# phymhan/supervised-gan

Measured on AMD Instinct MI355X. Metric: train-step images/sec, fcgan 512x512 bs=1/GPU, higher is better.
Workload: dtype f32 (bf16x3 MFMA); 1 GPU; fcgan deconv-G(ngf32, z 8x8x8) + 3x PatchGAN-D(ndf32, n_layers 3, scale 1/2/4) 512x512 bs=1, n_update_D=1 n_update_G=2, Adam, pool 50 (BASELINE configs[1] shape, fp32 compute); synthetic batches resident in HBM (ring of 64); parallelism=dp1, global_batch=1, hip_graph=True, skip_wasted_D_wgrad=False

## Files before the change

supervised-gan_amd/csrc/sgan_ew.hip:

```cpp
#include "sgan_reduce.h"

thread_local char g_sgan_err[512] = {0};
thread_local const char* g_sgan_last_kernel = "";

int sgan_fail(int code, const char* fmt, ...) {
    va_list ap;
    va_start(ap, fmt);
    vsnprintf(g_sgan_err, sizeof(g_sgan_err), fmt, ap);
    va_end(ap);
    return code;
}

extern "C" const char* sgan_version(void) { return "sgan_hip 0.2 (gfx950; fp32 MFMA 16x16x4 + split-bf16 MFMA 32x32x16)"; }
extern "C" const char* sgan_last_error(void) { return g_sgan_err; }
extern "C" const char* sgan_last_kernel(void) { return g_sgan_last_kernel; }
extern "C" int sgan_stat_replicas(void) { return SGAN_STAT_REPLICAS; }
extern "C" int sgan_set_device(int32_t device_id) {
    hipError_t e = hipSetDevice(device_id);
    if (e != hipSuccess) {
        (void)hipGetLastError();
        return sgan_fail(SGAN_ERR_HIP, "hipSetDevice(%d): %s", (int)device_id, hipGetErrorString(e));
    }
    return SGAN_OK;
}
extern "C" int sgan_stream_device(void* stream, int32_t* device_id) {
    if (!device_id) return sgan_fail(SGAN_ERR_INVALID, "null device_id");
    hipDevice_t dev;
    hipError_t e = hipStreamGetDevice((hipStream_t)stream, &dev);
    if (e != hipSuccess) {
        (void)hipGetLastError();
        return sgan_fail(SGAN_ERR_HIP, "hipStreamGetDevice: %s", hipGetErrorString(e));
    }
    *device_id = (int32_t)dev;
    return SGAN_OK;
}

#define SG_PROF_MAX 8192
static bool g_prof_on = false;
static int g_prof_n = 0;
static hipEvent_t g_prof_e0[SG_PROF_MAX], g_prof_e1[SG_PROF_MAX];
static const char* g_prof_name[SG_PROF_MAX];
static bool g_prof_open = false;

void sg_prof_begin(hipStream_t st) {
    if (!g_prof_on || g_prof_n >= SG_PROF_MAX) return;
    if (hipEventCreate(&g_prof_e0[g_prof_n]) != hipSuccess || hipEventCreate(&g_prof_e1[g_prof_n]) != hipSuccess) return;
    (void)hipEventRecord(g_prof_e0[g_prof_n], st);
    g_prof_open = true;
}

void sg_prof_end(hipStream_t st, const char* name) {
    if (!g_prof_open) return;
    (void)hipEventRecord(g_prof_e1[g_prof_n], st);
    g_prof_name[g_prof_n] = name;
    ++g_prof_n;
    g_prof_open = false;
}

extern "C" int sgan_profile_enable(int on) {
    for (int i = 0; i < g_prof_n; ++i) {
        (void)hipEventDestroy(g_prof_e0[i]);
        (void)hipEventDestroy(g_prof_e1[i]);
    }
    g_prof_n = 0;
    g_prof_on = on != 0;
    return SGAN_OK;
}

extern "C" int sgan_profile_count(void) { return g_prof_n; }

extern "C" int sgan_profile_mark(void* stream) {
    sg_prof_begin((hipStream_t)stream);
    sg_prof_end((hipStream_t)stream, "null");
    return SGAN_OK;
}

extern "C" int sgan_profile_read(int i, const char** name, float* ms) {
    if (i < 0 || i >= g_prof_n || !name || !ms) return sgan_fail(SGAN_ERR_INVALID, "bad profile record index");
    *name = g_prof_name[i];
    if (hipEventElapsedTime(ms, g_prof_e0[i], g_prof_e1[i]) != hipSuccess) return sgan_fail(SGAN_ERR_HIP, "hipEventElapsedTime failed");
    return SGAN_OK;
}

struct SgNormBwdJob {
    float* dy; const float* x; const double* sums; float* dgamma; float* dbeta; unsigned* amax;
    SgNorm xn;
    int32_t dy_ld, x_ld, npix, C, sums_sq, sums_rep, blocks;
};
struct SgNormBwdTable { SgNormBwdJob j[8]; };

__global__ __launch_bounds__(256) void sg_norm_bwd_apply_kernel(const SgNormBwdTable T) {
    sg_warm_kernargs<(int)sizeof(SgNormBwdTable)>();
    const SgNormBwdJob& J = T.j[blockIdx.y];
    if ((int)blockIdx.x >= J.blocks) return;
    const int C = J.C;
    extern __shared__ __attribute__((aligned(16))) char smem[];
    float* cA = reinterpret_cast<float*>(smem);
    float* cMean = cA + C;
    float* cRstd = cMean + C;
    float* cS1 = cRstd + C;
    float* cS2 = cS1 + C;
    const double invM = 1.0 / (double)J.npix;
    for (int c = threadIdx.x; c < C; c += 256) {
        float mean, rstd;
        sg_mean_rstd(J.xn, C, c, mean, rstd);
        const float g = J.xn.gamma ? J.xn.gamma[c] : 1.f;
        cA[c] = g * rstd;
        cMean[c] = mean;
        cRstd[c] = rstd;
        const double s1 = sg_stat_sum(J.sums, c, J.sums_rep), s2 = sg_stat_sum(J.sums, J.sums_sq + c, J.sums_rep);
        cS1[c] = (float)(s1 * invM);
        cS2[c] = (float)(s2 * invM);
        if (blockIdx.x == 0) {
            if (J.dgamma) atomicAdd(&J.dgamma[c], (float)s2);
            if (J.dbeta) atomicAdd(&J.dbeta[c], (float)s1);
        }
    }
    SG_SYNC();
    const int CQ = C >> 2;
    const int64_t total = (int64_t)J.npix * CQ;
    float* dy = J.dy;
    const float* x = J.x;
    const int64_t stride = (int64_t)J.blocks * 256;
    float amax = 0.f;
    for (int64_t e0 = (int64_t)blockIdx.x * 256 + threadIdx.x; e0 < total; e0 += 4 * stride) {
        f32x4 d[4], xv[4];
        int64_t od[4];
        int cc[4];
#pragma unroll
        for (int u = 0; u < 4; ++u) {
            const int64_t e = e0 + u * stride;
            const bool ok = e < total;
            const int p = ok ? (int)(e / CQ) : 0;
            cc[u] = ok ? (int)(e - (int64_t)p * CQ) * 4 : 0;
            od[u] = ok ? (int64_t)p * J.dy_ld + cc[u] : -1;
            d[u] = *reinterpret_cast<const f32x4*>(dy + (ok ? od[u] : 0));
            xv[u] = *reinterpret_cast<const f32x4*>(x + (ok ? (int64_t)p * J.x_ld + cc[u] : 0));
        }
#pragma unroll
        for (int u = 0; u < 4; ++u) {
            if (od[u] < 0) continue;
            const int c = cc[u];
#pragma unroll
            for (int j = 0; j < 4; ++j) {
                const float xhat = (xv[u][j] - cMean[c + j]) * cRstd[c + j];
                d[u][j] = cA[c + j] * (d[u][j] - cS1[c + j] - xhat * cS2[c + j]);
                amax = fmaxf(amax, fabsf(d[u][j]));
            }
            *reinterpret_cast<f32x4*>(dy + od[u]) = d[u];
        }
    }
    if (J.amax) {
        for (int o = 32; o > 0; o >>= 1) amax = fmaxf(amax, __shfl_xor(amax, o));
        SG_SYNC();
        if ((threadIdx.x & 63) == 0) cA[threadIdx.x >> 6] = amax;
        SG_SYNC();
        if (threadIdx.x == 0) {
            const unsigned mine = __builtin_bit_cast(unsigned, fmaxf(fmaxf(cA[0], cA[1]), fmaxf(cA[2], cA[3])));
            if (mine > __hip_atomic_load(J.amax, __ATOMIC_RELAXED, __HIP_MEMORY_SCOPE_AGENT)) atomicMax(J.amax, mine);
        }
    }
}

extern "C" int sgan_norm_bwd_apply_multi(const sgan_norm_bwd_job* jobs, int32_t n, void* stream) {
    SGAN_CHECK(jobs && n >= 1 && n <= 8, "1..8 jobs");
    SgNormBwdTable T;
    int maxb = 1, maxC = 4;
    for (int i = 0; i < n; ++i) {
        const sgan_norm_bwd_job& S = jobs[i];
        SGAN_CHECK(S.dy && S.x && S.x_norm && S.x_norm->stats && S.bwd_sums, "null argument in job %d", i);
        SGAN_CHECK((S.C & 3) == 0 && S.C > 0 && S.C <= 4096 && S.dy_ld >= S.C && S.x_ld >= S.C && (S.dy_ld & 3) == 0 &&
                       (S.x_ld & 3) == 0 && S.npix > 0, "bad dims in job %d", i);
        SgNormBwdJob& J = T.j[i];
        J.dy = S.dy; J.x = S.x; J.sums = S.bwd_sums; J.dgamma = S.dgamma; J.dbeta = S.dbeta;
        J.amax = reinterpret_cast<unsigned*>(S.amax_out);
        J.xn = sg_norm_from(S.x_norm);
        J.dy_ld = S.dy_ld; J.x_ld = S.x_ld; J.npix = S.npix; J.C = S.C;
        J.sums_sq = S.bwd_sums_sq_stride ? S.bwd_sums_sq_stride : S.C;
        J.sums_rep = S.bwd_sums_rep_stride;
        const int64_t total = (int64_t)S.npix * (S.C >> 2);
        static const int chunk = getenv("SGAN_NBA_CHUNK") ? atoi(getenv("SGAN_NBA_CHUNK")) : 4;
        int blocks = sg_cdiv(total, 256 * (chunk > 0 ? chunk : 4));
        if (blocks > 2048) blocks = 2048;
        if (blocks < 1) blocks = 1;
        J.blocks = blocks;
        if (blocks > maxb) maxb = blocks;
        if (S.C > maxC) maxC = S.C;
    }
    hipLaunchKernelGGL(sg_norm_bwd_apply_kernel, dim3(maxb, n), dim3(256), (size_t)5 * maxC * 4, (hipStream_t)stream, T);
    SGAN_LAUNCH_CHECK();
    return SGAN_OK;
}

extern "C" int sgan_norm_bwd_apply(float* dy, int32_t dy_ld, const float* x, int32_t x_ld, int32_t npix, int32_t C,
                                   const sgan_norm_desc* x_norm, const double* bwd_sums, int32_t bwd_sums_sq_stride,
                                   float* dgamma, float* dbeta, void* stream) {
    sgan_norm_bwd_job j = {dy, dy_ld, x, x_ld, npix, C, x_norm, bwd_sums, bwd_sums_sq_stride, dgamma, dbeta, 0, nullptr};
    return sgan_norm_bwd_apply_multi(&j, 1, stream);
}

__global__ __launch_bounds__(256) void sg_norm_apply_fwd_kernel(const float* u, int u_ld, SgNorm un, const float* mask,
                                                                const float* noise, float sigma, float* t, int t_ld, int npix,
                                                                int C) {
    extern __shared__ __attribute__((aligned(16))) char smem[];
    float* cMean = reinterpret_cast<float*>(smem);
    float* cA = cMean + C;
    float* cB = cA + C;
    for (int c = threadIdx.x; c < C; c += 256) {
        float mean = 0.f, rstd = 1.f;
        if (un.stats) sg_mean_rstd(un, C, c, mean, rstd);
        cMean[c] = mean;
        cA[c] = (un.gamma ? un.gamma[c] : 1.f) * rstd;
        cB[c] = un.beta ? un.beta[c] : 0.f;
    }
    SG_SYNC();
    const int CQ = C >> 2;
    const int64_t total = (int64_t)npix * CQ;
    for (int64_t e = (int64_t)blockIdx.x * 256 + threadIdx.x; e < total; e += (int64_t)gridDim.x * 256) {
        const int p = (int)(e / CQ), c = (int)(e - (int64_t)p * CQ) * 4;
        const f32x4 x = *reinterpret_cast<const f32x4*>(u + (int64_t)p * u_ld + c);
        f32x4 m = (f32x4){1.f, 1.f, 1.f, 1.f}, nz = (f32x4){0.f, 0.f, 0.f, 0.f};
        if (mask) m = *reinterpret_cast<const f32x4*>(mask + (int64_t)p * C + c);
        if (noise) nz = *reinterpret_cast<const f32x4*>(noise + (int64_t)p * C + c);
        f32x4 o;
#pragma unroll
        for (int j = 0; j < 4; ++j) o[j] = ((x[j] - cMean[c + j]) * cA[c + j] + cB[c + j]) * m[j] + sigma * nz[j];
        *reinterpret_cast<f32x4*>(t + (int64_t)p * t_ld + c) = o;
    }
}

__global__ __launch_bounds__(256) void sg_norm_apply_bwd_sums_kernel(float* dt, int dt_ld, const float* mask, const float* u,
                                                                     int u_ld, SgNorm un, double* sums, int npix, int C) {
    extern __shared__ __attribute__((aligned(16))) char smem[];
    float* cMean = reinterpret_cast<float*>(smem);
    float* cRstd = cMean + C;
    float* red = cRstd + C;
    for (int c = threadIdx.x; c < C; c += 256) {
        float mean = 0.f, rstd = 1.f;
        if (un.stats) sg_mean_rstd(un, C, c, mean, rstd);
        cMean[c] = mean;
        cRstd[c] = rstd;
    }
    for (int i = threadIdx.x; i < 2 * C; i += 256) red[i] = 0.f;
    SG_SYNC();
    const int CQ = C >> 2;
    const int64_t total = (int64_t)npix * CQ;
    if (256 % CQ == 0) {
        const int c = (threadIdx.x % CQ) * 4;
        const f32x4 mean = *reinterpret_cast<const f32x4*>(cMean + c), rstd = *reinterpret_cast<const f32x4*>(cRstd + c);
        f32x4 s1 = (f32x4){0.f, 0.f, 0.f, 0.f}, s2 = s1;
        for (int64_t e = (int64_t)blockIdx.x * 256 + threadIdx.x; e < total; e += (int64_t)gridDim.x * 256) {
            const int64_t p = e / CQ;
            f32x4 d = *reinterpret_cast<const f32x4*>(dt + p * dt_ld + c);
            const f32x4 x = *reinterpret_cast<const f32x4*>(u + p * u_ld + c);
            if (mask) {
                d *= *reinterpret_cast<const f32x4*>(mask + p * C + c);
                *reinterpret_cast<f32x4*>(dt + p * dt_ld + c) = d;
            }
            s1 += d;
            s2 += d * ((x - mean) * rstd);
        }
#pragma unroll
        for (int j = 0; j < 4; ++j) {
            atomicAdd(&red[c + j], s1[j]);
            atomicAdd(&red[C + c + j], s2[j]);
        }
    } else {
        for (int64_t e = (int64_t)blockIdx.x * 256 + threadIdx.x; e < total; e += (int64_t)gridDim.x * 256) {
            const int p = (int)(e / CQ), c = (int)(e - (int64_t)p * CQ) * 4;
            f32x4 d = *reinterpret_cast<const f32x4*>(dt + (int64_t)p * dt_ld + c);
            const f32x4 x = *reinterpret_cast<const f32x4*>(u + (int64_t)p * u_ld + c);
            if (mask) {
                const f32x4 m = *reinterpret_cast<const f32x4*>(mask + (int64_t)p * C + c);
                d *= m;
                *reinterpret_cast<f32x4*>(dt + (int64_t)p * dt_ld + c) = d;
            }
#pragma unroll
            for (int j = 0; j < 4; ++j) {
                const float xhat = (x[j] - cMean[c + j]) * cRstd[c + j];
                atomicAdd(&red[c + j], d[j]);
                atomicAdd(&red[C + c + j], d[j] * xhat);
            }
        }
    }
    SG_SYNC();
    for (int c = threadIdx.x; c < C; c += 256) {
        atomicAdd(&sums[c], (double)red[c]);
        atomicAdd(&sums[C + c], (double)red[C + c]);
    }
}

extern "C" int sgan_norm_apply_fwd(const float* u, int32_t u_ld, const sgan_norm_desc* u_norm, const float* mask,
                                   const float* noise, float sigma, float* t, int32_t t_ld, int32_t npix, int32_t C, void* stream) {
    SGAN_CHECK(u && t && npix > 0 && C > 0 && (C & 3) == 0 && u_ld >= C && t_ld >= C && (u_ld & 3) == 0 && (t_ld & 3) == 0, "bad argument");
    const int64_t total = (int64_t)npix * (C >> 2);
    int blocks = sg_cdiv(total, 256 * 2);
    if (blocks > 2048) blocks = 2048;
    if (blocks < 1) blocks = 1;
    hipLaunchKernelGGL(sg_norm_apply_fwd_kernel, dim3(blocks), dim3(256), (size_t)3 * C * 4, (hipStream_t)stream, u, u_ld,
                       sg_norm_from(u_norm), mask, noise, sigma, t, t_ld, npix, C);
    SGAN_LAUNCH_CHECK();
    return SGAN_OK;
}

extern "C" int sgan_norm_apply_bwd_sums(float* dt, int32_t dt_ld, const float* mask, const float* u, int32_t u_ld,
                                        const sgan_norm_desc* u_norm, double* bwd_sums, int32_t npix, int32_t C, void* stream) {
    SGAN_CHECK(dt && u && bwd_sums && npix > 0 && C > 0 && (C & 3) == 0 && u_ld >= C && dt_ld >= C, "bad argument");
    const int64_t total = (int64_t)npix * (C >> 2);
    int blocks = sg_cdiv(total, 256 * 8);
    if (blocks > 512) blocks = 512;
    if (blocks < 1) blocks = 1;
    hipLaunchKernelGGL(sg_norm_apply_bwd_sums_kernel, dim3(blocks), dim3(256), (size_t)4 * C * 4, (hipStream_t)stream, dt, dt_ld,
                       mask, u, u_ld, sg_norm_from(u_norm), bwd_sums, npix, C);
    SGAN_LAUNCH_CHECK();
    return SGAN_OK;
}

__device__ __forceinline__ int sg_refl(int i, int n) { return i < 0 ? -i : (i >= n ? 2 * (n - 1) - i : i); }

__global__ __launch_bounds__(256) void sg_pad_reflect_fwd_kernel(const float* x, int x_ld, int H, int W, int C, SgNorm xn, const float* mask,
                                                                 int pad, float* out, int out_ld) {
    extern __shared__ __attribute__((aligned(16))) char smem[];
    float* cSc = reinterpret_cast<float*>(smem);
    float* cSh = cSc + C;
    for (int c = threadIdx.x; c < C; c += 256) {
        float sc = 1.f, sh = 0.f;
        if (xn.stats) {
            float mean, rstd;
            sg_mean_rstd(xn, C, c, mean, rstd);
            const float gm = xn.gamma ? xn.gamma[c] : 1.f, bt = xn.beta ? xn.beta[c] : 0.f;
            sc = gm * rstd;
            sh = bt - mean * sc;
        }
        cSc[c] = sc;
        cSh[c] = sh;
    }
    SG_SYNC();
    const int CQ = C >> 2, Wp = W + 2 * pad, Hp = H + 2 * pad;
    const int64_t total = (int64_t)Hp * Wp * CQ;
    for (int64_t e = (int64_t)blockIdx.x * 256 + threadIdx.x; e < total; e += (int64_t)gridDim.x * 256) {
        const int c = (int)(e % CQ) * 4;
        const int64_t pp = e / CQ;
        const int px = (int)(pp % Wp), py = (int)(pp / Wp);
        const int64_t src = (int64_t)sg_refl(py - pad, H) * W + sg_refl(px - pad, W);
        f32x4 v = *reinterpret_cast<const f32x4*>(x + src * x_ld + c);
#pragma unroll
        for (int j = 0; j < 4; ++j) v[j] = sg_act(v[j] * cSc[c + j] + cSh[c + j], xn.act, xn.slope);
        if (mask) v *= *reinterpret_cast<const f32x4*>(mask + src * C + c);
        *reinterpret_cast<f32x4*>(out + pp * out_ld + c) = v;
    }
}

extern "C" int sgan_pad_reflect_fwd(const float* x, int32_t x_ld, int32_t H, int32_t W, int32_t C, const sgan_norm_desc* x_norm,
                                    const float* mask, int32_t pad, float* out, int32_t out_ld, void* stream) {
    SGAN_CHECK(x && out && H > 0 && W > 0 && C > 0 && (C & 3) == 0 && (x_ld & 3) == 0 && (out_ld & 3) == 0 && x_ld >= C && out_ld >= C,
               "bad argument");
    SGAN_CHECK(pad >= 0 && pad < H && pad < W, "reflection padding must be smaller than the image");
    const int64_t total = (int64_t)(H + 2 * pad) * (W + 2 * pad) * (C >> 2);
    int blocks = sg_cdiv(total, 256 * 4);
    if (blocks > 2048) blocks = 2048;
    hipLaunchKernelGGL(sg_pad_reflect_fwd_kernel, dim3(blocks), dim3(256), (size_t)2 * C * 4, (hipStream_t)stream, x, x_ld, H, W, C,
                       sg_norm_from(x_norm), mask, pad, out, out_ld);
    SGAN_LAUNCH_CHECK();
    return SGAN_OK;
}

__global__ __launch_bounds__(256) void sg_pad_reflect_bwd_kernel(const float* dout, int dout_ld, int H, int W, int C, int pad, const float* x,
                                                                 int x_ld, SgNorm xn, const float* mask, float* din, int din_ld,
                                                                 double* sums, int sums_sq) {
    extern __shared__ __attribute__((aligned(16))) char smem[];
    float* cMean = reinterpret_cast<float*>(smem);
    float* cRstd = cMean + C;
    float* cG = cRstd + C;
    float* cB = cG + C;
    double* red = reinterpret_cast<double*>(cB + C);
    for (int c = threadIdx.x; c < C; c += 256) {
        float mean = 0.f, rstd = 1.f;
        if (xn.stats) sg_mean_rstd(xn, C, c, mean, rstd);
        cMean[c] = mean;
        cRstd[c] = rstd;
        cG[c] = (xn.stats && xn.gamma) ? xn.gamma[c] : 1.f;
        cB[c] = (xn.stats && xn.beta) ? xn.beta[c] : 0.f;
    }
    for (int i = threadIdx.x; i < 2 * C; i += 256) red[i] = 0.0;
    SG_SYNC();
    const int CQ = C >> 2, Wp = W + 2 * pad;
    const int64_t total = (int64_t)H * W * CQ;
    const bool has_x = x != nullptr;
    for (int64_t e = (int64_t)blockIdx.x * 256 + threadIdx.x; e < total; e += (int64_t)gridDim.x * 256) {
        const int c = (int)(e % CQ) * 4;
        const int64_t pix = e / CQ;
        const int xx = (int)(pix % W), yy = (int)(pix / W);
        int ys[3], xs[3], ny = 0, nx = 0;
        ys[ny++] = yy + pad;
        if (yy >= 1 && yy <= pad) ys[ny++] = pad - yy;
        if (yy <= H - 2 && yy >= H - 1 - pad) ys[ny++] = pad + 2 * (H - 1) - yy;
        xs[nx++] = xx + pad;
        if (xx >= 1 && xx <= pad) xs[nx++] = pad - xx;
        if (xx <= W - 2 && xx >= W - 1 - pad) xs[nx++] = pad + 2 * (W - 1) - xx;
        f32x4 d = (f32x4){0.f, 0.f, 0.f, 0.f};
        for (int a = 0; a < ny; ++a)
            for (int b = 0; b < nx; ++b) d += *reinterpret_cast<const f32x4*>(dout + ((int64_t)ys[a] * Wp + xs[b]) * dout_ld + c);
        if (mask) d *= *reinterpret_cast<const f32x4*>(mask + pix * C + c);
        if (has_x) {
            const f32x4 xv = *reinterpret_cast<const f32x4*>(x + pix * x_ld + c);
#pragma unroll
            for (int j = 0; j < 4; ++j) {
                const float xhat = (xv[j] - cMean[c + j]) * cRstd[c + j];
                const float y = xn.stats ? cG[c + j] * xhat + cB[c + j] : xv[j];
                d[j] *= sg_act_grad(y, xn.act, xn.slope);
                if (sums) {
                    atomicAdd(&red[c + j], (double)d[j]);
                    atomicAdd(&red[C + c + j], (double)(d[j] * xhat));
                }
            }
        }
        *reinterpret_cast<f32x4*>(din + pix * din_ld + c) = d;
    }
    if (sums) {
        SG_SYNC();
        for (int c = threadIdx.x; c < C; c += 256) {
            atomicAdd(&sums[c], red[c]);
            atomicAdd(&sums[(sums_sq ? sums_sq : C) + c], red[C + c]);
        }
    }
}

extern "C" int sgan_pad_reflect_bwd(const float* dout, int32_t dout_ld, int32_t H, int32_t W, int32_t C, int32_t pad, const float* x,
                                    int32_t x_ld, const sgan_norm_desc* x_norm, const float* mask, float* din, int32_t din_ld,
                                    double* bwd_sums, int32_t bwd_sums_sq_stride, void* stream) {
    SGAN_CHECK(dout && din && H > 0 && W > 0 && C > 0 && (C & 3) == 0 && (dout_ld & 3) == 0 && (din_ld & 3) == 0 && dout_ld >= C && din_ld >= C,
               "bad argument");
    SGAN_CHECK(pad >= 0 && 2 * pad < H && 2 * pad < W, "reflection padding must be smaller than half the image");
    SGAN_CHECK(!(bwd_sums && !x), "bwd_sums needs x");
    SGAN_CHECK(!x || ((x_ld & 3) == 0 && x_ld >= C), "bad x_ld");
    const int64_t total = (int64_t)H * W * (C >> 2);
    int blocks = sg_cdiv(total, 256 * 4);
    if (blocks > 1024) blocks = 1024;
    hipLaunchKernelGGL(sg_pad_reflect_bwd_kernel, dim3(blocks), dim3(256), (size_t)4 * C * 4 + (size_t)2 * C * 8, (hipStream_t)stream, dout,
                       dout_ld, H, W, C, pad, x, x_ld, sg_norm_from(x ? x_norm : nullptr), mask, din, din_ld, bwd_sums, bwd_sums_sq_stride);
    SGAN_LAUNCH_CHECK();
    return SGAN_OK;
}

#define SG_IMGLOSS_BLOCKS 256
__device__ __forceinline__ void sg_block_partial(double acc, double* part) {
    __shared__ double wsum[4];
    const double sum = sg_block_sum<4>(acc, wsum);
    if (threadIdx.x == 0) part[blockIdx.x] = sum;
}

__global__ __launch_bounds__(64) void sg_imgloss_fin_kernel(const double* part, int nparts, double scale, float* loss_out) {
    double acc = 0.0;
    for (int i = threadIdx.x; i < nparts; i += 64) acc += part[i];
    acc = sg_wave_sum(acc);
    if (threadIdx.x == 0) loss_out[0] = (float)(acc * scale);
}

__global__ __launch_bounds__(256) void sg_l1w_fwd_kernel(const float* x, int x_ld, const float* y, int y_ld, int npix, int C,
                                                         const float* a, int a_ld, const float* wts, int nw, float lambda,
                                                         double* part, float* g, int g_ld) {
    const double inv = 1.0 / ((double)npix * (double)C);
    double acc = 0.0;
    for (int p = blockIdx.x * 256 + threadIdx.x; p < npix; p += gridDim.x * 256) {
        float w = 1.f;
        if (a) {
            if (nw == 0) w = a[(int64_t)p * a_ld];
            for (int i = 0; i < nw; ++i) w += (a[(int64_t)p * a_ld + i] + 1.f) * 0.5f * (wts[i] - 1.f);
        }
        for (int c = 0; c < g_ld; ++c) {
            float gv = 0.f;
            if (c < C) {
                const float d = x[(int64_t)p * x_ld + c] - y[(int64_t)p * y_ld + c];
                acc += (double)(fabsf(d) * w);
                gv = (d > 0.f ? 1.f : (d < 0.f ? -1.f : 0.f)) * w * lambda * (float)inv;
            }
            g[(int64_t)p * g_ld + c] = gv;
        }
    }
    sg_block_partial(acc, part);
}

__global__ __launch_bounds__(256) void sg_scale_kernel(const float* gout, const float* g, float* dx, int64_t n4) {
    const float s = gout[0];
    for (int64_t e = (int64_t)blockIdx.x * 256 + threadIdx.x; e < n4; e += (int64_t)gridDim.x * 256) {
        f32x4 v = reinterpret_cast<const f32x4*>(g)[e];
        v *= s;
        reinterpret_cast<f32x4*>(dx)[e] = v;
    }
}

__global__ __launch_bounds__(256) void sg_bce01_fwd_kernel(const float* x, int x_ld, const float* t, int t_ld, int npix, int C,
// ... 1701 lines not shown
```

Before: 515.1 images/sec.

## Pack norm-backward jobs into flat grid and prefetch loads before stat setup

The multi-job norm backward apply kernel now launches a flat 1-D grid with per-job prefix block offsets, so no empty blocks are spawned when jobs have unequal sizes. The first batch of dy/x loads is issued before the per-channel mean/rstd/stat shared-memory setup, so that latency overlaps. Index math switches from 64-bit division per element to incremental 32-bit (p,q) stepping. Jobs with npix*C/4 of 2^31 or more are now rejected, and the larger table adds kernarg size.

```diff
diff --git a/supervised-gan_amd/csrc/sgan_ew.hip b/supervised-gan_amd/csrc/sgan_ew.hip
--- a/supervised-gan_amd/csrc/sgan_ew.hip
+++ b/supervised-gan_amd/csrc/sgan_ew.hip
@@ -87,12 +87,18 @@
     SgNorm xn;
     int32_t dy_ld, x_ld, npix, C, sums_sq, sums_rep, blocks;
 };
-struct SgNormBwdTable { SgNormBwdJob j[8]; };
+struct SgNormBwdTable { SgNormBwdJob j[8]; int32_t first[8]; };
+
+#define SG_NBA_UNROLL 4
 
 __global__ __launch_bounds__(256) void sg_norm_bwd_apply_kernel(const SgNormBwdTable T) {
     sg_warm_kernargs<(int)sizeof(SgNormBwdTable)>();
-    const SgNormBwdJob& J = T.j[blockIdx.y];
-    if ((int)blockIdx.x >= J.blocks) return;
+    const int bid = (int)blockIdx.x;
+    int ji = 0;
+#pragma unroll
+    for (int i = 1; i < 8; ++i) ji += bid >= T.first[i];
+    const SgNormBwdJob& J = T.j[ji];
+    const int lb = bid - T.first[ji];
     const int C = J.C;
     extern __shared__ __attribute__((aligned(16))) char smem[];
     float* cA = reinterpret_cast<float*>(smem);
@@ -100,6 +106,33 @@
     float* cRstd = cMean + C;
     float* cS1 = cRstd + C;
     float* cS2 = cS1 + C;
+    const uint32_t CQ = (uint32_t)C >> 2;
+    const uint32_t total = (uint32_t)J.npix * CQ;
+    const uint32_t stride = (uint32_t)J.blocks * 256u;
+    const uint32_t sp = stride / CQ, sq = stride - sp * CQ;
+    float* dy = J.dy;
+    const float* x = J.x;
+    const int64_t dy_ld = J.dy_ld, x_ld = J.x_ld;
+    uint32_t e = (uint32_t)lb * 256u + threadIdx.x;
+    uint32_t p = e / CQ, q = e - p * CQ;
+    f32x4 d[SG_NBA_UNROLL], xv[SG_NBA_UNROLL];
+    int64_t od[SG_NBA_UNROLL];
+    int cc[SG_NBA_UNROLL];
+    auto load_trip = [&]() {
+#pragma unroll
+        for (int u = 0; u < SG_NBA_UNROLL; ++u) {
+            const bool ok = e < total;
+            cc[u] = (int)q * 4;
+            od[u] = ok ? (int64_t)p * dy_ld + cc[u] : -1;
+            if (ok) {
+                d[u] = *reinterpret_cast<const f32x4*>(dy + od[u]);
+                xv[u] = *reinterpret_cast<const f32x4*>(x + (int64_t)p * x_ld + cc[u]);
+            }
+            e += stride; p += sp; q += sq;
+            if (q >= CQ) { q -= CQ; ++p; }
+        }
+    };
+    load_trip();
     const double invM = 1.0 / (double)J.npix;
     for (int c = threadIdx.x; c < C; c += 256) {
         float mean, rstd;
@@ -111,34 +144,16 @@
         const double s1 = sg_stat_sum(J.sums, c, J.sums_rep), s2 = sg_stat_sum(J.sums, J.sums_sq + c, J.sums_rep);
         cS1[c] = (float)(s1 * invM);
         cS2[c] = (float)(s2 * invM);
-        if (blockIdx.x == 0) {
+        if (lb == 0) {
             if (J.dgamma) atomicAdd(&J.dgamma[c], (float)s2);
             if (J.dbeta) atomicAdd(&J.dbeta[c], (float)s1);
         }
     }
     SG_SYNC();
-    const int CQ = C >> 2;
-    const int64_t total = (int64_t)J.npix * CQ;
-    float* dy = J.dy;
-    const float* x = J.x;
-    const int64_t stride = (int64_t)J.blocks * 256;
     float amax = 0.f;
-    for (int64_t e0 = (int64_t)blockIdx.x * 256 + threadIdx.x; e0 < total; e0 += 4 * stride) {
-        f32x4 d[4], xv[4];
-        int64_t od[4];
-        int cc[4];
-#pragma unroll
-        for (int u = 0; u < 4; ++u) {
-            const int64_t e = e0 + u * stride;
-            const bool ok = e < total;
-            const int p = ok ? (int)(e / CQ) : 0;
-            cc[u] = ok ? (int)(e - (int64_t)p * CQ) * 4 : 0;
-            od[u] = ok ? (int64_t)p * J.dy_ld + cc[u] : -1;
-            d[u] = *reinterpret_cast<const f32x4*>(dy + (ok ? od[u] : 0));
-            xv[u] = *reinterpret_cast<const f32x4*>(x + (ok ? (int64_t)p * J.x_ld + cc[u] : 0));
-        }
-#pragma unroll
-        for (int u = 0; u < 4; ++u) {
+    for (;;) {
+#pragma unroll
+        for (int u = 0; u < SG_NBA_UNROLL; ++u) {
             if (od[u] < 0) continue;
             const int c = cc[u];
 #pragma unroll
@@ -149,6 +164,8 @@
             }
             *reinterpret_cast<f32x4*>(dy + od[u]) = d[u];
         }
+        if (e >= total) break;
+        load_trip();
     }
     if (J.amax) {
         for (int o = 32; o > 0; o >>= 1) amax = fmaxf(amax, __shfl_xor(amax, o));
@@ -165,12 +182,16 @@
 extern "C" int sgan_norm_bwd_apply_multi(const sgan_norm_bwd_job* jobs, int32_t n, void* stream) {
     SGAN_CHECK(jobs && n >= 1 && n <= 8, "1..8 jobs");
     SgNormBwdTable T;
-    int maxb = 1, maxC = 4;
+    int maxC = 4;
+    int64_t totals[8];
+    for (int i = 0; i < 8; ++i) T.first[i] = INT32_MAX;
     for (int i = 0; i < n; ++i) {
         const sgan_norm_bwd_job& S = jobs[i];
         SGAN_CHECK(S.dy && S.x && S.x_norm && S.x_norm->stats && S.bwd_sums, "null argument in job %d", i);
         SGAN_CHECK((S.C & 3) == 0 && S.C > 0 && S.C <= 4096 && S.dy_ld >= S.C && S.x_ld >= S.C && (S.dy_ld & 3) == 0 &&
                        (S.x_ld & 3) == 0 && S.npix > 0, "bad dims in job %d", i);
+        totals[i] = (int64_t)S.npix * (S.C >> 2);
+        if (totals[i] >= (1ll << 31)) return sgan_fail(SGAN_ERR_UNSUPPORTED, "norm backward: npix * C / 4 >= 2^31 (job %d)", i);
         SgNormBwdJob& J = T.j[i];
         J.dy = S.dy; J.x = S.x; J.sums = S.bwd_sums; J.dgamma = S.dgamma; J.dbeta = S.dbeta;
         J.amax = reinterpret_cast<unsigned*>(S.amax_out);
@@ -178,16 +199,19 @@
         J.dy_ld = S.dy_ld; J.x_ld = S.x_ld; J.npix = S.npix; J.C = S.C;
         J.sums_sq = S.bwd_sums_sq_stride ? S.bwd_sums_sq_stride : S.C;
         J.sums_rep = S.bwd_sums_rep_stride;
-        const int64_t total = (int64_t)S.npix * (S.C >> 2);
-        static const int chunk = getenv("SGAN_NBA_CHUNK") ? atoi(getenv("SGAN_NBA_CHUNK")) : 4;
-        int blocks = sg_cdiv(total, 256 * (chunk > 0 ? chunk : 4));
+        if (S.C > maxC) maxC = S.C;
+    }
+    static const int chunk_env = getenv("SGAN_NBA_CHUNK") ? atoi(getenv("SGAN_NBA_CHUNK")) : 0;
+    const int chunk = chunk_env > 0 ? chunk_env : SG_NBA_UNROLL;
+    int nblocks = 0;
+    for (int i = 0; i < n; ++i) {
+        int blocks = sg_cdiv(totals[i], 256 * chunk);
         if (blocks > 2048) blocks = 2048;
-        if (blocks < 1) blocks = 1;
-        J.blocks = blocks;
-        if (blocks > maxb) maxb = blocks;
-        if (S.C > maxC) maxC = S.C;
-    }
-    hipLaunchKernelGGL(sg_norm_bwd_apply_kernel, dim3(maxb, n), dim3(256), (size_t)5 * maxC * 4, (hipStream_t)stream, T);
+        T.j[i].blocks = blocks;
+        T.first[i] = nblocks;
+        nblocks += blocks;
+    }
+    hipLaunchKernelGGL(sg_norm_bwd_apply_kernel, dim3(nblocks), dim3(256), (size_t)5 * maxC * 4, (hipStream_t)stream, T);
     SGAN_LAUNCH_CHECK();
     return SGAN_OK;
 }
```

Result: no change. 517.0 images/sec, median of 6 (+0.4%).
